# lunarlab-gatech/SLIDE_SLAM

Hardware: AMD Instinct MI355X
Metric: pose-graph updates/sec + ms/Gauss-Newton iter, 8-robot 10k-landmark graph (higher is better)
Workload: dtype f64

## Files before the change

slide_slam_amd/csrc/chol_kernels.hip:

```cpp
#include <hip/hip_runtime.h>
#include <stdlib.h>
#include <algorithm>
#include <type_traits>
#include <utility>
#include <vector>

#include "graph_dev.hpp"
#include "kernels.hpp"

namespace sl {

typedef double v4d __attribute__((ext_vector_type(4)));
constexpr int CHOL_BATCH_MAX = 8;
__device__ inline v4d mfma_f64(double a, double b, v4d c) { return __builtin_amdgcn_mfma_f64_16x16x4f64(a, b, c, 0, 0, 0); }

__device__ inline double rsqrt_nr(double d) {
#ifdef SLIDE_RSQRT_OLD
  double y = __builtin_amdgcn_rsq(d);
  y = y * (1.5 - 0.5 * d * y * y);
  y = y * (1.5 - 0.5 * d * y * y);
  return y;
#else
  double y = __builtin_amdgcn_rsq(d);
  double t = d * y, h = 0.5 * y;
// ... 1712 lines not shown
  }
}

extern "C" int slide_debug_pair_timeouts() {
  int v = -1;
  if (hipMemcpyFromSymbol(&v, HIP_SYMBOL(g_pair_timeouts), sizeof(int)) != hipSuccess) return -1;
  return v;
}
#ifdef SLIDE_STAMPS
extern "C" void slide_debug_stamps(unsigned long long* out) { (void)hipMemcpyFromSymbol(out, HIP_SYMBOL(g_stamps), sizeof(g_stamps)); }
extern "C" void slide_debug_chain_stamps(unsigned long long* out) { (void)hipMemcpyFromSymbol(out, HIP_SYMBOL(g_chain_stamps), sizeof(g_chain_stamps)); }
#endif

constexpr unsigned long long BWD_SENT = CHAIN_SENTINEL;

__global__ void k_chol_extract_y(const double* __restrict__ S, int ld, int T, int Tr, double* __restrict__ yv, double* __restrict__ dp, int* status,
                                 double* __restrict__ prev) {
  const int c = blockIdx.x * blockDim.x + threadIdx.x;
  if (c == 0) status[4] = 0;
  if (c < T * NB) {
    yv[c] = S[(size_t)c * ld + (size_t)Tr * NB];
    if (prev) prev[c] = dp[c];
    dp[c] = __longlong_as_double((long long)BWD_SENT);
  }
}

struct ExtractArgs { int n; const double* S[CHOL_STEP_BATCH_MAX]; int ld[CHOL_STEP_BATCH_MAX]; int T[CHOL_STEP_BATCH_MAX]; int Tr[CHOL_STEP_BATCH_MAX]; double* yv[CHOL_STEP_BATCH_MAX]; double* dp[CHOL_STEP_BATCH_MAX]; int* status[CHOL_STEP_BATCH_MAX]; };
__global__ void k_chol_extract_y_b(ExtractArgs A) {
  const int r = blockIdx.y;
  const int c = blockIdx.x * blockDim.x + threadIdx.x;
  if (c == 0) A.status[r][4] = 0;
  if (c < A.T[r] * NB) {
    A.yv[r][c] = A.S[r][(size_t)c * A.ld[r] + (size_t)A.Tr[r] * NB];
    A.dp[r][c] = __longlong_as_double((long long)BWD_SENT);
  }
}

constexpr int CHAIN_THREADS = 320;
struct alignas(16) ChainLds {
// ... 599 lines not shown
                            hipStream_t s) {
  const int nT = T * NB;
  for (int k = row0 / NB; k < T; ++k)
    hipLaunchKernelGGL(k_cov_fwd, dim3((unsigned)(T - k)), dim3(256), 0, s, S, ld, k, Ld + (size_t)k * NB * NB, Winv + (size_t)k * 1024, Y, nT);
  hipLaunchKernelGGL(k_cov_gram, dim3(1), dim3(256), 0, s, Y, nT, row0 / NB * NB, cov36);
}

struct SyrkArgs {
  int n;
  const double* S[CHOL_BATCH_MAX]; int ld[CHOL_BATCH_MAX]; int T[CHOL_BATCH_MAX]; int nbr[CHOL_BATCH_MAX];
  int b0[CHOL_BATCH_MAX];
  double* bord[CHOL_BATCH_MAX]; int ldb[CHOL_BATCH_MAX]; const int* bfirst[CHOL_BATCH_MAX];
  const double* bsrc[CHOL_BATCH_MAX];
  int ks; double* scratch;
  size_t scratch_stride;
  int ks_sys[2];
  const int* jobs;
  const int* segtab[CHOL_BATCH_MAX];
};
template <int RD>
__device__ __forceinline__ void border_syrk_body(const SyrkArgs& A) {
  int r = A.ks > 1 ? 0 : blockIdx.z, ib = blockIdx.x, jb = blockIdx.y;
  const int q = A.ks > 1 ? blockIdx.z : 0;
  if (A.jobs) {
    const int j = A.jobs[blockIdx.x];
    r = j >> 20; ib = (j >> 10) & 1023; jb = j & 1023;
  }
  const int nbr = A.nbr[r];
  if (ib > nbr || jb >= nbr || ib < jb) return;
  const int T = A.T[r], ld = A.ld[r];
  int ldb = A.ldb[r];
  int c0 = 0, c1 = T;
  const int* st = A.segtab[r];
  const int nseg = st ? st[0] : 1;
  if (!st && A.bfirst[r]) c0 = max(A.bfirst[r][ib], A.bfirst[r][jb]);
  int ksr = A.ks;
  if (A.ks > 1) {
    if (A.scratch_stride && r < 2 && A.ks_sys[r] > 0) ksr = A.ks_sys[r];
    if (q >= ksr) return;
    const int len = (T - c0 + ksr - 1) / ksr;
    c0 += q * len;
    c1 = min(T, c0 + len);
  }
  const double* bsrc = A.bsrc[r];
  if (!st && c0 >= c1 && !(bsrc && q == 0)) return;
  const double* S = A.S[r];
  const int wq = threadIdx.x >> 6, lane = threadIdx.x & 63, lr = lane & 15, lk = lane >> 4;
  const int ch = (wq >> 1) & 1, rh = wq & 1;
  if (A.jobs && ib == nbr && rh == 1 && !bsrc) return;
  const int B0 = A.b0[r];
  const double* pj0 = S + (size_t)lk * ld + (size_t)(B0 + jb) * NB + 32 * ch + 2 * lr;
  const double* pi0 = S + (size_t)lk * ld + (size_t)(B0 + ib) * NB + 32 * rh + 2 * lr;
  double* cbh = A.bord[r] + (size_t)(jb * NB + 32 * ch + 2 * lk) * ldb + (size_t)ib * NB + 32 * rh + 2 * lr;
  const double* cin = bsrc ? bsrc + (size_t)(jb * NB + 32 * ch + 2 * lk) * ldb + (size_t)ib * NB + 32 * rh + 2 * lr : cbh;
  const int ldin = ldb;
  if (q > 0) {
    ldb = NB;
    cbh = A.scratch + (size_t)r * A.scratch_stride + ((size_t)(jb * (nbr + 1) + ib) * (ksr - 1) + (q - 1)) * (NB * NB) + (size_t)(32 * ch + 2 * lk) * NB + 32 * rh + 2 * lr;
  }
  int total = 0;
  if (st) {
    for (int sg = 0; sg < nseg; ++sg) {
      const int* sf = st + 1 + nseg + sg * (nbr + 1);
      const int a0 = max(sf[ib], sf[jb]), a1 = st[1 + sg];
      if (a0 < a1) total += (a1 - a0) * 16;
    }
  } else {
    total = c1 > c0 ? (c1 - c0) * 16 : 0;
  }
  int sg_next = 0, rem = 0, issued = 0;
  const double *lpj = pj0, *lpi = pi0;
  v2d pa[RD], pb[RD];
  auto issue = [&](v2d& ra, v2d& rb) {
// ... 51 lines not shown
    for (int e = 0; e < 4; ++e) {
      v2d c2;
      c2[0] = acc[a][0][e]; c2[1] = acc[a][1][e];
      *(v2d*)(cbh + (size_t)(8 * e + a) * ldb) = c2;
    }
}
__global__ __launch_bounds__(256) void k_border_syrk(SyrkArgs A) { border_syrk_body<16>(A); }
__global__ __launch_bounds__(256) void k_border_syrk_rd8(SyrkArgs A) { border_syrk_body<8>(A); }
__global__ __launch_bounds__(256) void k_border_syrk_rd4(SyrkArgs A) { border_syrk_body<4>(A); }
static void launch_syrk_kernel(dim3 grid, size_t lds, hipStream_t s, const SyrkArgs& A) {
  static const int rd = getenv("SLIDE_SYRK_RD") ? atoi(getenv("SLIDE_SYRK_RD")) : 16;
  if (rd == 4) hipLaunchKernelGGL(k_border_syrk_rd4, grid, dim3(256), lds, s, A);
  else if (rd == 8) hipLaunchKernelGGL(k_border_syrk_rd8, grid, dim3(256), lds, s, A);
  else hipLaunchKernelGGL(k_border_syrk, grid, dim3(256), lds, s, A);
}
__global__ __launch_bounds__(256) void k_border_syrk_reduce(double* __restrict__ bord, int ldb, int nbr, int ks, const double* __restrict__ scratch,
                                                            const int* __restrict__ bfirst, int T) {
  const int ib = blockIdx.x >> 4, jb = blockIdx.y;
  if (ib > nbr || jb >= nbr || ib < jb) return;
  int c0 = 0;
  if (bfirst) c0 = max(bfirst[ib], bfirst[jb]);
  const int len = (T - c0 + ks - 1) / ks;
  const int e = (blockIdx.x & 15) * 256 + threadIdx.x;
  const int col = e / NB, row = e - col * NB;
  double* dst = bord + (size_t)(jb * NB + col) * ldb + (size_t)ib * NB + row;
  double v = *dst;
  for (int q = 1; q < ks; ++q)
    if (c0 + q * len < T) v += scratch[((size_t)(jb * (nbr + 1) + ib) * (ks - 1) + (q - 1)) * (NB * NB) + (size_t)col * NB + row];
  *dst = v;
}
__global__ __launch_bounds__(256) void k_border_syrk_reduce2(double* __restrict__ bordA, int ldbA, const double* __restrict__ bordB, int ldbB, int nbr,
                                                             int ksA, int ksB, const double* __restrict__ scratchA, const double* __restrict__ scratchB,
                                                             int TA, int TB) {
  const int ib = blockIdx.x >> 4, jb = blockIdx.y;
  if (ib > nbr || jb >= nbr || ib < jb) return;
  const int e = (blockIdx.x & 15) * 256 + threadIdx.x;
  const int col = e / NB, row = e - col * NB;
  double* dst = bordA + (size_t)(jb * NB + col) * ldbA + (size_t)ib * NB + row;
  double va = *dst, vb = bordB[(size_t)(jb * NB + col) * ldbB + (size_t)ib * NB + row];
  const int lenA = (TA + ksA - 1) / ksA, lenB = (TB + ksB - 1) / ksB;
  for (int q = 1; q < ksA; ++q)
    if (q * lenA < TA) va += scratchA[((size_t)(jb * (nbr + 1) + ib) * (ksA - 1) + (q - 1)) * (NB * NB) + (size_t)col * NB + row];
  for (int q = 1; q < ksB; ++q)
    if (q * lenB < TB) vb += scratchB[((size_t)(jb * (nbr + 1) + ib) * (ksB - 1) + (q - 1)) * (NB * NB) + (size_t)col * NB + row];
  *dst = va + vb;
}
void launch_border_syrk(const CholSystem* d, int n, hipStream_t s, double* scratch, int ks) {
  SyrkArgs A{};
  A.n = n;
  int nb = 0;
  for (int i = 0; i < n; ++i) {
    A.S[i] = d[i].S; A.ld[i] = d[i].ld; A.T[i] = d[i].T; A.nbr[i] = d[i].nbr; A.bord[i] = d[i].bord; A.ldb[i] = d[i].ldb; A.bfirst[i] = d[i].bfirst; A.bsrc[i] = d[i].bord_src;
    A.segtab[i] = d[i].segtab; A.b0[i] = d[i].b0 > 0 ? d[i].b0 : d[i].T;
    nb = d[i].nbr > nb ? d[i].nbr : nb;
  }
  if (nb <= 0) return;
  if (scratch && n == 1 && ks > 1) {
    A.ks = ks; A.scratch = scratch;
    launch_syrk_kernel(dim3(nb + 1, nb, ks), 0, s, A);
    hipLaunchKernelGGL(k_border_syrk_reduce, dim3(16 * (nb + 1), nb), dim3(256), 0, s, d[0].bord, d[0].ldb, d[0].nbr, ks, scratch, d[0].bfirst, d[0].T);
    return;
  }
  A.ks = 1; A.scratch = nullptr;
  launch_syrk_kernel(dim3(nb + 1, nb, n), 0, s, A);
}
void launch_border_syrk_jobs(const CholSystem* d, int n, const int* jobs, int njobs, int lds_pad, hipStream_t s, double* scratch, int ks, int jb_end,
                             const int* ks_sys, bool fuse_add) {
  SyrkArgs A{};
  A.n = n;
  for (int i = 0; i < n; ++i) {
    A.S[i] = d[i].S; A.ld[i] = d[i].ld; A.T[i] = d[i].T; A.nbr[i] = d[i].nbr; A.bord[i] = d[i].bord; A.ldb[i] = d[i].ldb; A.bfirst[i] = d[i].bfirst; A.bsrc[i] = d[i].bord_src;
    A.segtab[i] = d[i].segtab; A.b0[i] = d[i].b0 > 0 ? d[i].b0 : d[i].T;
  }
  if (njobs <= 0) return;
  A.ks = 1; A.scratch = nullptr; A.jobs = jobs;
// ... 3 lines not shown
    A.ks = km; A.scratch = scratch; A.scratch_stride = std::max<size_t>(1, (size_t)(nb + 1) * nb * (km - 1) * NB * NB);
    A.ks_sys[0] = ka; A.ks_sys[1] = kb;
    launch_syrk_kernel(dim3(njobs, 1, km), lds_pad, s, A);
    hipLaunchKernelGGL(k_border_syrk_reduce2, dim3(16 * (nb + 1), jb_end >= 0 ? jb_end : nb), dim3(256), 0, s, d[0].bord, d[0].ldb, d[1].bord, d[1].ldb, nb,
                       ka, kb, scratch, scratch + A.scratch_stride, d[0].T, d[1].T);
    return;
  }
  if (scratch && n == 1 && ks > 1) {
    A.ks = ks; A.scratch = scratch;
    launch_syrk_kernel(dim3(njobs, 1, ks), lds_pad, s, A);
    const int nb = d[0].nbr;
    hipLaunchKernelGGL(k_border_syrk_reduce, dim3(16 * (nb + 1), jb_end >= 0 ? jb_end : nb), dim3(256), 0, s, d[0].bord, d[0].ldb, nb, ks, scratch, d[0].bfirst, d[0].T);
    return;
  }
  launch_syrk_kernel(dim3(njobs), lds_pad, s, A);
}
struct BorderApplyArgs {
  int n;
  const double* S[CHOL_BATCH_MAX]; int ld[CHOL_BATCH_MAX]; int T[CHOL_BATCH_MAX]; int nbr[CHOL_BATCH_MAX]; int b0[CHOL_BATCH_MAX];
  double* yv[CHOL_BATCH_MAX]; const double* x[CHOL_BATCH_MAX];
  const int* segtab[CHOL_BATCH_MAX];
};
__global__ __launch_bounds__(256) void k_border_apply(BorderApplyArgs A) {
  const int r = blockIdx.z;
  const int col = blockIdx.x * 4 + (threadIdx.x >> 6), lane = threadIdx.x & 63;
  if (col >= A.T[r] * NB) return;
  const int nrow = A.nbr[r] * NB;
  const double* w = A.S[r] + (size_t)col * A.ld[r] + (size_t)A.b0[r] * NB;
  const double* x = A.x[r];
  double acc = 0.0;
// ... 491 lines not shown
```

slide_slam_amd/csrc/host_graph.hip:

```cpp
#include <chrono>

#include "host_graph.hpp"

#include <algorithm>
#include <cmath>
#include <cstdio>
#include <cstdlib>
#include <map>
#include <unordered_map>

namespace sl {

static inline int lam_ks_cap(int nl) {
  const int tiles = (nl + 1) * nl;
  if (tiles <= 0) return 1;
  return tiles <= 32 ? 16 : std::max(1, std::min(16, 256 / tiles));
}

thread_local std::string g_last_error;
void thread_capture_mode_local() {
  thread_local bool done = false;
  if (done) return;
  hipStreamCaptureMode m = hipStreamCaptureModeThreadLocal;
  (void)hipThreadExchangeStreamCaptureMode(&m);
// ... 777 lines not shown
  c.Ld = sep_Ld + (size_t)TL * NB * NB; c.Winv = sep_Winv + (size_t)TL * 1024; c.yv = sep_yv + (size_t)TL * NB; c.dp = sep_dp + (size_t)TL * NB;
  c.status = sep_status; c.nbr = sep_nl;
  if (!sep_dissected() && sep_prof_on) c.h_prof = h_sep_prof.data();
  return c;
}
void CholBatch::free_separator() {
  free_ll_sep_plans();
  if (sepS) (void)hipFree(sepS);
  sepS = nullptr; sep_len = 0;
  for (double** p : {&sep_Ld, &sep_Winv, &sep_yv, &sep_dp, &sep_bord, &lamS, &lam_Ld, &lam_Winv, &lam_yv, &lam_dp, &lam_scratch}) if (*p) { (void)hipFree(*p); *p = nullptr; }
  for (int** p : {&sep_status, &sep_ctr, &d_sep_off, &lam_status, &lam_ctr, &d_sep_prof, &d_leaf_prof, &sep_ctr2, &d_sep_jobs, &d_sep_tmask}) if (*p) { (void)hipFree(*p); *p = nullptr; }
  if (sep_scratch) { (void)hipFree(sep_scratch); sep_scratch = nullptr; }
  for (double** p : {&sep_top2, &sep_bord2}) if (*p) { (void)hipFree(*p); *p = nullptr; }
  if (d_sep_jobs2) { (void)hipFree(d_sep_jobs2); d_sep_jobs2 = nullptr; }
  if (d_lam_jobs2) { (void)hipFree(d_lam_jobs2); d_lam_jobs2 = nullptr; }
  sep_cap = 0; lam_cap = -1;
}
void CholBatch::set_segments(int n) {
  std::lock_guard<std::mutex> pl(pass_mtx);
  exact_serial = 0;
  std::vector<HostGraph*> gs;
  {
    std::lock_guard<std::mutex> lk(mtx);
    n_seg = n < 1 ? 1 : (n > 8 ? 8 : n);
    pass_dirty = true;
    gs.assign(graphs.begin(), graphs.end());
  }
  for (HostGraph* g : gs)
    if (g) { std::lock_guard<std::mutex> gl(g->mtx); g->topo_dirty = true; }
}
// ... 154 lines not shown
    for (int jb = 0; jb < Tt; ++jb)
      for (int ib = jb; ib <= nb; ++ib) codes.push_back(ib << 10 | jb);
    n_sep_jobs = (int)codes.size();
    SL_HIP(hipMalloc(reinterpret_cast<void**>(&d_sep_jobs), codes.size() * sizeof(int)));
    SL_HIP(hipMemcpyAsync(d_sep_jobs, codes.data(), codes.size() * sizeof(int), hipMemcpyHostToDevice, master)); SL_HIP(hipStreamSynchronize(master));
    sep_ks = std::max(1, std::min({8, TL / 4, (1024 + n_sep_jobs - 1) / std::max(n_sep_jobs, 1)}));
    if (getenv("SLIDE_SEP_KS")) sep_ks = std::max(1, std::min(16, atoi(getenv("SLIDE_SEP_KS"))));
    {
      std::vector<int> codes2;
      for (int sy = 0; sy < 2; ++sy)
        for (int c : codes) codes2.push_back(sy << 20 | c);
      if (d_sep_jobs2) { SL_HIP(hipFree(d_sep_jobs2)); d_sep_jobs2 = nullptr; }
      n_sep_jobs2 = (int)codes2.size();
      SL_HIP(hipMalloc(reinterpret_cast<void**>(&d_sep_jobs2), codes2.size() * sizeof(int)));
      SL_HIP(hipMemcpyAsync(d_sep_jobs2, codes2.data(), codes2.size() * sizeof(int), hipMemcpyHostToDevice, master)); SL_HIP(hipStreamSynchronize(master));
    }
    if (sep_ks > 1) {
      const size_t len = 2 * (size_t)(nb + 1) * nb * (sep_ks - 1) * NB * NB * sizeof(double);
      SL_HIP(hipMalloc(reinterpret_cast<void**>(&sep_scratch), len));
      SL_HIP(hipMemsetAsync(sep_scratch, 0, len, master)); SL_HIP(hipStreamSynchronize(master));
    }
    for (double** p : {&sep_top2, &sep_bord2}) if (*p) { SL_HIP(hipFree(*p)); *p = nullptr; }
    sep_ld2 = (Tt + sep_nl + 1) * NB;
    SL_HIP(hipMalloc(reinterpret_cast<void**>(&sep_top2), (size_t)sep_ld2 * Tt * NB * sizeof(double)));
    SL_HIP(hipMemsetAsync(sep_top2, 0, (size_t)sep_ld2 * Tt * NB * sizeof(double), master));
    if (sep_nl > 0) {
      const size_t nb2 = (size_t)(sep_nl + 1) * NB * sep_nl * NB;
      SL_HIP(hipMalloc(reinterpret_cast<void**>(&sep_bord2), nb2 * sizeof(double)));
      SL_HIP(hipMemsetAsync(sep_bord2, 0, nb2 * sizeof(double), master));
    }
// ... 147 lines not shown
          CholSystem tp2[2] = {top, top};
          for (int hh = 0; hh < 2; ++hh) {
            tp2[hh].S = sepS + (size_t)(hh ? sTa : 0) * NB * ld_s; tp2[hh].T = sep_leafT[hh]; tp2[hh].b0 = sTL;
            if (hh) { tp2[hh].bord = sep_top2; tp2[hh].ldb = sep_ld2; }
          }
          CholSystem sl2[2];
          int ks_lam[2] = {1, 1};
          for (int hh = 0; hh < 2 && sep_nl > 0; ++hh) {
            CholSystem sl{};
            sl.S = sepS + (size_t)(hh ? sTa : 0) * NB * ld_s; sl.ld = ld_s; sl.T = sep_leafT[hh]; sl.b0 = sep_Ts; sl.nbr = sep_nl;
            sl.bord = hh ? sep_bord2 : sep_bord; sl.ldb = (sep_nl + 1) * NB;
            ks_lam[hh] = std::max(1, std::min(lam_ks_cap(sep_nl), sep_leafT[hh] / 2));
            sl2[hh] = sl;
          }
          if (sep_scratch && (sep_nl == 0 || (lam_scratch && d_lam_jobs2))) {
            launch_border_syrk_jobs(tp2, 2, d_sep_jobs2, n_sep_jobs2, 0, master, sep_scratch, sep_ks, Tt, nullptr, true);
            if (sep_nl > 0) launch_border_syrk_jobs(sl2, 2, d_lam_jobs2, n_lam_jobs2, 0, master, lam_scratch, 1, -1, ks_lam, true);
          } else {
            for (int hh = 0; hh < 2; ++hh) {
              launch_border_syrk_jobs(&tp2[hh], 1, d_sep_jobs, n_sep_jobs, 0, master, sep_scratch, sep_ks, Tt);
              if (sep_nl > 0) launch_border_syrk(&sl2[hh], 1, master, lam_scratch, ks_lam[hh]);
            }
            launch_sep_top_add(Y, sTL, sep_top2, sep_ld2, sep_bord2, master);
          }
        } else {
          launch_border_syrk_jobs(&top, 1, d_sep_jobs, n_sep_jobs, 0, master, sep_scratch, sep_ks, Tt);
        }
      }
      if (ll_top) {
        const CholSystem ts = sep_top_system();
        launch_chol_ll(ll_top, &ts, 1, master);
      } else if ((chol_pair_mask() & 8) && d_pair_tickets) {
// ... 12 lines not shown
      const CholSystem ts = sep_top_system();
      launch_chol_batch(&ts, 1, sep_ctr, master, nullptr, false, 100, pair_tickets(11));
    } else {
      for (int k = 0; k < sep_Ts; ++k)
        launch_chol_step(sepS, ld_s, k, sep_Ts, sep_Ld + (size_t)k * NB * NB, sep_Winv + (size_t)k * 1024, sep_status, sep_ctr, nullptr,
                         sep_prof_on ? h_sep_prof.data() : nullptr, master, sep_nl);
      launch_chol_extract_y(sepS, ld_s, sep_Ts, sep_yv, sep_dp, sep_status, master, sep_nl);
    }
    if (sep_nl > 0) {
      CholSystem ss{};
      ss.S = sepS; ss.ld = ld_s; ss.T = sep_Ts; ss.yv = sep_yv; ss.nbr = sep_nl; ss.bord = sep_bord; ss.ldb = (sep_nl + 1) * NB; ss.bfirst = nullptr;
      CholSystem sr = ss;
      static const bool env_canon3 = !(getenv("SLIDE_SEP_CANONICAL") && getenv("SLIDE_SEP_CANONICAL")[0] == '0');
      if (owned || (whole && sep_dissected() && env_canon3 && n <= 8)) { sr.S = sepS + (size_t)sTL * NB * ld_s; sr.T = sTt; sr.b0 = sep_Ts; }
      const int ks = std::max(1, std::min(lam_ks_cap(sep_nl), sr.T / 2));
      launch_border_syrk(&sr, 1, master, lam_scratch, ks);
      launch_lam_prepare(sep_bord, sep_nl, sep_lam, lamS, master);
      const int ld_l = (sep_nl + 1) * NB;
      for (int k = 0; k < sep_nl; ++k)
        launch_chol_step(lamS, ld_l, k, sep_nl, lam_Ld + (size_t)k * NB * NB, lam_Winv + (size_t)k * 1024, lam_status, lam_ctr, nullptr, nullptr, master);
      launch_chol_extract_y(lamS, ld_l, sep_nl, lam_yv, lam_dp, lam_status, master);
      launch_chol_bwd_all(lamS, ld_l, sep_nl, lam_Ld, lam_Winv, lam_yv, lam_dp, lam_status, nullptr, master);
      const double* xl = lam_dp;
      if (!owned) launch_border_apply(&ss, 1, &xl, master);
      else {
        CholSystem ap2[2] = {ss, ss};
        ap2[0].S = sepS + (size_t)own_t0 * NB * ld_s; ap2[0].T = own_T; ap2[0].b0 = sep_Ts; ap2[0].yv = sep_yv + (size_t)own_t0 * NB;
        ap2[1].S = sepS + (size_t)sTL * NB * ld_s; ap2[1].T = sTt; ap2[1].b0 = sep_Ts; ap2[1].yv = sep_yv + (size_t)sTL * NB;
        const double* xl2[2] = {xl, xl};
        launch_border_apply(ap2, 2, xl2, master);
      }
    }
    if (sep_dissected()) {
      double* St = sepS + (size_t)sTL * NB * ld_s + (size_t)sTL * NB;
      launch_chol_bwd_all(St, ld_s, sTt, sep_Ld + (size_t)sTL * NB * NB, sep_Winv + (size_t)sTL * 1024, sep_yv + (size_t)sTL * NB, sep_dp + (size_t)sTL * NB,
                          sep_status, nullptr, master);
      launch_ints_clear(sep_status + 4, 1, master);
// ... 1689 lines not shown
```

slide_slam_amd/csrc/host_graph.hpp:

```cpp
#pragma once
#include <hip/hip_runtime.h>

#include <cstdint>
#include <cstring>
#include <condition_variable>
#include <functional>
#include <mutex>
#include <string>
#include <unordered_map>
#include <vector>

#include "../../include/slide_gpu.h"
#include "graph_dev.hpp"
#include "host_layout.hpp"
#include "kernels.hpp"
#include "sl_math.hpp"

namespace sl {

extern thread_local std::string g_last_error;
void thread_capture_mode_local();
bool hip_ok(hipError_t e, const char* what);
inline bool robot_ok(int r) { return r >= 0 && r < SLIDE_MAX_ROBOTS; }
int decode_status(const int* st8);
// ... 222 lines not shown
  double* sep_x = nullptr; long long sep_x_len = 0;
  int sep_m = 0, sep_Ts = 0;
  double *sep_Ld = nullptr, *sep_Winv = nullptr, *sep_yv = nullptr, *sep_dp = nullptr;
  int *sep_status = nullptr, *sep_ctr = nullptr, *d_sep_off = nullptr;
  int sep_cap = 0;
  std::vector<int> h_sep_prof; int* d_sep_prof = nullptr; bool sep_prof_on = false;
  int sep_leafT[2] = {0, 0}, sep_used[2] = {0, 0};
  int sep_owner = -1; bool sep_leader = true;
  std::vector<int> h_leaf_prof[2];
  int* d_leaf_prof = nullptr;
  int* d_sep_tmask = nullptr;
  int* sep_ctr2 = nullptr; int* d_sep_jobs = nullptr; int n_sep_jobs = 0; double* sep_scratch = nullptr; int sep_ks = 1;
  double *sep_top2 = nullptr, *sep_bord2 = nullptr; int sep_ld2 = 0; unsigned sep_mask_b = 0;
  int* d_lam_jobs2 = nullptr; int n_lam_jobs2 = 0;
  int* d_sep_jobs2 = nullptr; int n_sep_jobs2 = 0;
  bool sep_dissected() const { return sep_leafT[0] > 0 && sep_leafT[1] > 0; }
  int sep_lam = 0, sep_nl = 0, lam_cap = -1;
  double *lam_scratch = nullptr;
  double *sep_bord = nullptr, *lamS = nullptr, *lam_Ld = nullptr, *lam_Winv = nullptr, *lam_yv = nullptr, *lam_dp = nullptr;
  int *lam_status = nullptr, *lam_ctr = nullptr;
  SepLayout sep_layout() const {
    SepLayout Y{sepS, sep_bord, sep_x, sep_Ts, sep_nl, sep_m, sep_lam, {0, 0, 0, 0}, 0, 0};
    if (sep_dissected()) {
      Y.gap[0] = sep_used[0]; Y.gap[1] = sep_leafT[0] * NB;
      Y.gap[2] = sep_leafT[0] * NB + sep_used[1]; Y.gap[3] = (sep_leafT[0] + sep_leafT[1]) * NB;
      Y.hTa = sep_leafT[0]; Y.hTL = sep_leafT[0] + sep_leafT[1];
    }
    return Y;
  }
  int prepare_separator();
// ... 391 lines not shown
```

slide_slam_amd/csrc/kernels.hpp:

```cpp
#pragma once
#include <hip/hip_runtime.h>
#include <stdint.h>
#include <vector>

#include "graph_dev.hpp"
#include "sl_math.hpp"

namespace sl {

void init_solver_kernels();
void launch_relin(const GraphDev& G, hipStream_t s);
void launch_linearize(const GraphDev& G, const ObsLossDev& O, hipStream_t s);
void launch_observation_weights(const GraphDev& G, const ObsLossDev& O, bool robust, int n, double* out2n, hipStream_t s);
void launch_observation_weights_batched(const GraphDev* d, const ObsLossDev* dO, bool robust, const int* off, const int* cnt, int n, double* out2n,
                                        hipStream_t s);
void launch_robust_reweight(const GraphDev& G, const RobustDev& R, hipStream_t s);
void launch_closure_weights(const GraphDev& G, const RobustDev& R, const int* idx, int n, double* out2n, hipStream_t s);
void launch_robust_reweight_batched(const GraphDev* d, const RobustDev* dR, const GraphDev* h, int n, hipStream_t s);
void launch_closure_weights_batched(const GraphDev* d, const RobustDev* dR, const int* ent2, int n, double* out2n, hipStream_t s);
void launch_landmark(const GraphDev& G, int mode, hipStream_t s);
void launch_pose(const GraphDev& G, hipStream_t s);
void launch_schur(const GraphDev& G, hipStream_t s);
void launch_backsub(const GraphDev& G, int mode, hipStream_t s);
void launch_shared_pack(const GraphDev& G, int what, double* buf, hipStream_t s);
// ... 15 lines not shown
void launch_phase2_batched(const GraphDev* d, const GraphDev* h, int n, double* const* bufs, hipStream_t s);
void launch_phase3_batched(const GraphDev* d, const GraphDev* h, int n, double* const* bufs, hipStream_t s);
void launch_ghost_exchange(const GraphDev& G, int what, double* buf, hipStream_t s);
void launch_ghost_exchange_batched(const GraphDev* d, int n, int n_gslots, int what, double* const* bufs, hipStream_t s);
void launch_border_assemble_batched(const GraphDev* d, const GraphDev* h, int n, hipStream_t s, bool clear = true, bool fills = true);
void launch_sep_extract_batched(const GraphDev* d, const GraphDev* h, int n, const int* n_sep_poses, hipStream_t s);
void launch_sep_pose_scatter_batched(const GraphDev* d, const GraphDev* h, int n, double* const* xloc, hipStream_t s);
struct SepLayout { double* sys; double* bord; double* packed; int Ts, nl, ms, lam; int gap[4]; int hTa, hTL; };
void launch_ghost_refresh_local(const GraphDev* d, int n, int n_gslots, hipStream_t s);
void launch_copy_pairs(const double* const* src, double* const* dst, const int* count, int n, hipStream_t s);
void launch_sep_gather(const GraphDev* h, int n, const int* const* maps, const SepLayout& Y, bool packed, hipStream_t s, const int* tmask = nullptr,
                       int split_col = -1, unsigned mask_b = 0, double* sys2 = nullptr, int ld2 = 0, double* bord2 = nullptr);
void launch_sep_top_add(const SepLayout& Y, int c0, const double* sys2, int ld2, const double* bord2, hipStream_t s);
void launch_sep_unpack(const SepLayout& Y, hipStream_t s, int c0 = 0, int c1 = -1, bool to_packed = false);
void launch_lam_prepare(const double* bord, int nl, int lam, double* out, hipStream_t s);
void launch_sep_xloc(int n, const int* const* maps, int ms, int lam, const double* xs, const double* xl, double* const* xloc, hipStream_t s);
void launch_arrow_finish_batched(const GraphDev* d, const GraphDev* h, int n, const double* xs, const int* sep_off, hipStream_t s, bool slots_onto);
struct AsmMerge { int mask; };
AsmMerge asm_merge_env();
void launch_phase3_arrow_batched(const GraphDev* d, const GraphDev* h, int n, hipStream_t s);

void launch_chol_step(double* S, int ld, int k, int T, double* Ld, double* Winv, int* status, int* ctr, float* L32, const int* h_prof, hipStream_t s, int nbr = 0);
void launch_chol_extract_y(const double* S, int ld, int T, double* yv, double* dp, int* status, hipStream_t s, int nbr = 0, int b0 = 0, double* prev = nullptr);
constexpr unsigned long long CHAIN_SENTINEL = 0x7FF8DEADBEEF0BADull;
struct CholSystem { double* S; int ld, T; double* Ld; double* Winv; double* yv; double* dp; int* status;
                    float* L32;
                    const int* h_prof;
                    const int* prof; const int* first;
                    double* ctab;
                    int nbr;
// ... 13 lines not shown
  ~CholPlanHook();
  CholPlanHook(const CholPlanHook&) = delete;
  CholPlanHook& operator=(const CholPlanHook&) = delete;
private:
  CholPlanHook* prev;
};
int chol_device_cus();
bool chol_pair_supported(const CholSystem* d, int n);
void launch_chol_bwd_batch(const CholSystem* d, int n, hipStream_t s);
struct CholLLPlan;
CholLLPlan* chol_ll_plan_create(const CholSystem* d, int n, const int* const* h_ord = nullptr, hipStream_t upload_stream = nullptr);
void chol_ll_plan_destroy(CholLLPlan* p);
int chol_ll_plan_tasks(const CholLLPlan* p);
int chol_ll_plan_columns(const CholLLPlan* p);
void launch_chol_ll(const CholLLPlan* p, const CholSystem* d, int n, hipStream_t s, int* trace = nullptr);
void launch_border_syrk(const CholSystem* d, int n, hipStream_t s, double* scratch = nullptr, int ks = 1);
void launch_border_syrk_jobs(const CholSystem* d, int n, const int* jobs, int njobs, int lds_pad, hipStream_t s, double* scratch = nullptr, int ks = 1, int jb_end = -1,
                             const int* ks_sys = nullptr, bool fuse_add = false);
void launch_border_apply(const CholSystem* d, int n, const double* const* xloc, hipStream_t s);
void launch_chain_batch(const CholSystem* d, int n, const double* const* in, double* const* out, bool fwd, bool f32, bool prepared,
                        double* const* next_out, hipStream_t s);
void launch_chain_tables(const CholSystem* d, int n, hipStream_t s);
void launch_chol_bwd_all(const double* S, int ld, int T, const double* Ld, const double* Winv, double* yv, double* dp, int* status, const int* prof, hipStream_t s,
                         const double* wf_prev = nullptr, double wf_thr = 0.0, int wf_Tprev = 0, int wf_lim = -1);
void launch_pose_covariance(const double* S, int ld, int T, const double* Ld, const double* Winv, double* Y, int row0, double* cov36,
                            hipStream_t s);
void launch_selected_inverse(const double* S, int ld, int T, const double* Ld, const double* Winv, const int* prof, const int* d_prof,
                             double* Sg, double* Z, hipStream_t s);
void launch_selected_inverse_prep(const double* S, int ld, int T, const double* Ld, const double* Winv, const int* prof, const int* d_prof,
                                  double* Sg, double* Z, hipStream_t s);
void launch_pose_blocks(const double* Sg, int ld, const int* poses, int n, double* out, hipStream_t s, const int* prow = nullptr);
void launch_landmark_covariances(const GraphDev& G, const double* Sg, int ld, const int* lids, int n, double* out, hipStream_t s,
                                 const int* prow = nullptr);
// ... 248 lines not shown
```

slide_slam_amd/csrc/solver_kernels.hip:

```cpp
#include <hip/hip_runtime.h>
#include <algorithm>
#include <cstring>

#include "graph_dev.hpp"
#include "kernels.hpp"
#include "sl_math.hpp"

namespace sl {

struct BufPtrs { double* p[8]; };

__device__ inline void pose_retract12(const double* in12, const double* d6, int chart, double* out12) {
  to12(retract(from12(in12), d6, chart), out12);
}
__device__ inline void lm_retract(int type, const double* in, const double* d, int chart, double* out) {
  if (type == VT_POINT) {
    out[0] = in[0] + d[0]; out[1] = in[1] + d[1]; out[2] = in[2] + d[2];
  } else if (type == VT_CUBE) {
    pose_retract12(in, d, chart, out);
    out[12] = in[12] + d[6]; out[13] = in[13] + d[7]; out[14] = in[14] + d[8];
  } else {
    out[3] = in[3] + d[0]; out[4] = in[4] + d[1]; out[5] = in[5] + d[2];
    out[0] = in[0] + d[3]; out[1] = in[1] + d[4]; out[2] = in[2] + d[5];
    out[6] = in[6] + d[6];
// ... 1563 lines not shown
      else A.bord2[(size_t)(vc - NL) * ((size_t)(Y.nl + 1) * NB) + (vr - NL)] = s2;
    }
  }
}
__global__ __launch_bounds__(256) void k_sep_unpack(SepLayout Y, int c0, int c1, int to_packed) {
  const int vr = blockIdx.x * 256 + threadIdx.x, vc = c0 * NB + blockIdx.y;
  const int NT = (Y.Ts + Y.nl) * NB;
  if (vr > NT || vc >= NT || vc >= c1 * NB || vr < vc / NB * NB) return;
  if (sep_packed_hole(vr, vc, Y.hTa, Y.hTL)) return;
  if (to_packed) { *sep_slot(Y, vr, vc, true) = *sep_slot(Y, vr, vc, false); return; }
  double v = *sep_slot(Y, vr, vc, true);
  if (vr == vc && ((vc >= Y.gap[0] && vc < Y.gap[1]) || (vc >= Y.gap[2] && vc < Y.gap[3]))) v = 1.0;
  *sep_slot(Y, vr, vc, false) = v;
}
__global__ __launch_bounds__(256) void k_lam_prepare(const double* __restrict__ bord, int nl, int lam, double* __restrict__ out) {
  const int r = blockIdx.x * 256 + threadIdx.x, c = blockIdx.y;
  const int NT = nl * NB, ld = (nl + 1) * NB;
  if (r > NT || c >= NT) return;
  const bool rhs = r == NT;
  if (!rhs && r < c) return;
  double v;
  if (c < lam && (rhs || r < lam)) v = -bord[(size_t)c * ld + r];
  else v = (r == c) ? 1.0 : 0.0;
  out[(size_t)c * ld + r] = v;
}
struct SepScatterArgs { int n, m, ms; const double* xs; const double* xl; double* xloc[8]; const int* map[8]; };
__global__ __launch_bounds__(256) void k_sep_xloc(SepScatterArgs A) {
  const int g = blockIdx.x * 256 + threadIdx.x, r = blockIdx.y;
  if (g >= A.m || r >= A.n) return;
  const int lc = A.map[r][g];
  if (lc >= 0) A.xloc[r][lc] = g < A.ms ? A.xs[g] : A.xl[g - A.ms];
}
__global__ __launch_bounds__(256) void k_sep_lm_delta_b(const GraphDev* __restrict__ Gs, SepScatterArgs A, const int* __restrict__ sep_off) {
  const GraphDev G = Gs[blockIdx.z];
  const int t = blockIdx.x * 256 + threadIdx.x;
  const int sidx = t / 9, k = t - 9 * sidx;
  if (sidx >= G.n_slots) return;
  const int l = G.sh_lid[sidx];
  if (l < 0) return;
// ... 585 lines not shown
```

Before: 4115.

## Fuse lambda-system syrk with top pairs and single-block lambda solve

Merges the border SYRK for the two top systems and the two lambda systems into one launch over a combined job list, with a paired reduce kernel handling both. For a one-block lambda system, the reduce, prepare, Cholesky step, y-extract and backward solve are folded into a single 512-thread kernel in place of a chain of small launches. The goal is to cut kernel-launch and serialization overhead on tiny systems. The cost is a single-block kernel with low parallelism and extra scratch indexing, both gated by an env mask that is on by default.

```diff
diff --git a/slide_slam_amd/csrc/chol_kernels.hip b/slide_slam_amd/csrc/chol_kernels.hip
--- a/slide_slam_amd/csrc/chol_kernels.hip
+++ b/slide_slam_amd/csrc/chol_kernels.hip
@@ -1750,15 +1750,18 @@
 
 constexpr unsigned long long BWD_SENT = CHAIN_SENTINEL;
 
-__global__ void k_chol_extract_y(const double* __restrict__ S, int ld, int T, int Tr, double* __restrict__ yv, double* __restrict__ dp, int* status,
-                                 double* __restrict__ prev) {
-  const int c = blockIdx.x * blockDim.x + threadIdx.x;
+__device__ __forceinline__ void extract_y_elem(const double* __restrict__ S, int ld, int T, int Tr, double* __restrict__ yv, double* __restrict__ dp,
+                                               int* status, double* __restrict__ prev, int c) {
   if (c == 0) status[4] = 0;
   if (c < T * NB) {
     yv[c] = S[(size_t)c * ld + (size_t)Tr * NB];
     if (prev) prev[c] = dp[c];
     dp[c] = __longlong_as_double((long long)BWD_SENT);
   }
+}
+__global__ void k_chol_extract_y(const double* __restrict__ S, int ld, int T, int Tr, double* __restrict__ yv, double* __restrict__ dp, int* status,
+                                 double* __restrict__ prev) {
+  extract_y_elem(S, ld, T, Tr, yv, dp, status, prev, blockIdx.x * blockDim.x + threadIdx.x);
 }
 
 struct ExtractArgs { int n; const double* S[CHOL_STEP_BATCH_MAX]; int ld[CHOL_STEP_BATCH_MAX]; int T[CHOL_STEP_BATCH_MAX]; int Tr[CHOL_STEP_BATCH_MAX]; double* yv[CHOL_STEP_BATCH_MAX]; double* dp[CHOL_STEP_BATCH_MAX]; int* status[CHOL_STEP_BATCH_MAX]; };
@@ -2388,7 +2391,8 @@
   const double* bsrc[CHOL_BATCH_MAX];
   int ks; double* scratch;
   size_t scratch_stride;
-  int ks_sys[2];
+  int ks_sys[4];
+  double* scratch2; size_t scratch_stride2;
   const int* jobs;
   const int* segtab[CHOL_BATCH_MAX];
 };
@@ -2410,7 +2414,7 @@
   if (!st && A.bfirst[r]) c0 = max(A.bfirst[r][ib], A.bfirst[r][jb]);
   int ksr = A.ks;
   if (A.ks > 1) {
-    if (A.scratch_stride && r < 2 && A.ks_sys[r] > 0) ksr = A.ks_sys[r];
+    if (A.scratch_stride && r < 4 && A.ks_sys[r] > 0) ksr = A.ks_sys[r];
     if (q >= ksr) return;
     const int len = (T - c0 + ksr - 1) / ksr;
     c0 += q * len;
@@ -2430,7 +2434,8 @@
   const int ldin = ldb;
   if (q > 0) {
     ldb = NB;
-    cbh = A.scratch + (size_t)r * A.scratch_stride + ((size_t)(jb * (nbr + 1) + ib) * (ksr - 1) + (q - 1)) * (NB * NB) + (size_t)(32 * ch + 2 * lk) * NB + 32 * rh + 2 * lr;
+    double* sc = r < 2 ? A.scratch + (size_t)r * A.scratch_stride : A.scratch2 + (size_t)(r - 2) * A.scratch_stride2;
+    cbh = sc + ((size_t)(jb * (nbr + 1) + ib) * (ksr - 1) + (q - 1)) * (NB * NB) + (size_t)(32 * ch + 2 * lk) * NB + 32 * rh + 2 * lr;
   }
   int total = 0;
   if (st) {
@@ -2512,27 +2517,51 @@
   else if (rd == 8) hipLaunchKernelGGL(k_border_syrk_rd8, grid, dim3(256), lds, s, A);
   else hipLaunchKernelGGL(k_border_syrk, grid, dim3(256), lds, s, A);
 }
-__global__ __launch_bounds__(256) void k_border_syrk_reduce(double* __restrict__ bord, int ldb, int nbr, int ks, const double* __restrict__ scratch,
-                                                            const int* __restrict__ bfirst, int T) {
-  const int ib = blockIdx.x >> 4, jb = blockIdx.y;
+template <int N>
+__device__ __forceinline__ void border_reduce_elems(double* __restrict__ bord, int ldb, int nbr, int ks, const double* __restrict__ scratch,
+                                                    const int* __restrict__ bfirst, int T, int ib, int jb, int e0, int stride) {
   if (ib > nbr || jb >= nbr || ib < jb) return;
   int c0 = 0;
   if (bfirst) c0 = max(bfirst[ib], bfirst[jb]);
   const int len = (T - c0 + ks - 1) / ks;
-  const int e = (blockIdx.x & 15) * 256 + threadIdx.x;
-  const int col = e / NB, row = e - col * NB;
-  double* dst = bord + (size_t)(jb * NB + col) * ldb + (size_t)ib * NB + row;
-  double v = *dst;
-  for (int q = 1; q < ks; ++q)
-    if (c0 + q * len < T) v += scratch[((size_t)(jb * (nbr + 1) + ib) * (ks - 1) + (q - 1)) * (NB * NB) + (size_t)col * NB + row];
-  *dst = v;
-}
-__global__ __launch_bounds__(256) void k_border_syrk_reduce2(double* __restrict__ bordA, int ldbA, const double* __restrict__ bordB, int ldbB, int nbr,
-                                                             int ksA, int ksB, const double* __restrict__ scratchA, const double* __restrict__ scratchB,
-                                                             int TA, int TB) {
-  const int ib = blockIdx.x >> 4, jb = blockIdx.y;
+  double* dst[N];
+  double v[N];
+#pragma unroll
+  for (int u = 0; u < N; ++u) {
+    const int e = e0 + u * stride;
+    const int col = e / NB, row = e - col * NB;
+    dst[u] = bord + (size_t)(jb * NB + col) * ldb + (size_t)ib * NB + row;
+    v[u] = *dst[u];
+  }
+  int nq = ks;
+  while (nq > 1 && c0 + (nq - 1) * len >= T) --nq;
+  const double* sq = scratch + (size_t)(jb * (nbr + 1) + ib) * (ks - 1) * (NB * NB) + e0;
+  int q = 1;
+  for (; q + 1 < nq; q += 2) {
+    double p[N], p2[N];
+#pragma unroll
+    for (int u = 0; u < N; ++u) { p[u] = sq[(size_t)(q - 1) * (NB * NB) + u * stride]; p2[u] = sq[(size_t)q * (NB * NB) + u * stride]; }
+#pragma unroll
+    for (int u = 0; u < N; ++u) { v[u] += p[u]; v[u] += p2[u]; }
+  }
+  if (q < nq) {
+    double p[N];
+#pragma unroll
+    for (int u = 0; u < N; ++u) p[u] = sq[(size_t)(q - 1) * (NB * NB) + u * stride];
+#pragma unroll
+    for (int u = 0; u < N; ++u) v[u] += p[u];
+  }
+#pragma unroll
+  for (int u = 0; u < N; ++u) *dst[u] = v[u];
+}
+__global__ __launch_bounds__(256) void k_border_syrk_reduce(double* __restrict__ bord, int ldb, int nbr, int ks, const double* __restrict__ scratch,
+                                                            const int* __restrict__ bfirst, int T) {
+  border_reduce_elems<1>(bord, ldb, nbr, ks, scratch, bfirst, T, blockIdx.x >> 4, blockIdx.y, (blockIdx.x & 15) * 256 + threadIdx.x, 0);
+}
+__device__ __forceinline__ void border_reduce2_elem(double* __restrict__ bordA, int ldbA, const double* __restrict__ bordB, int ldbB, int nbr,
+                                                    int ksA, int ksB, const double* __restrict__ scratchA, const double* __restrict__ scratchB,
+                                                    int TA, int TB, int ib, int jb, int e) {
   if (ib > nbr || jb >= nbr || ib < jb) return;
-  const int e = (blockIdx.x & 15) * 256 + threadIdx.x;
   const int col = e / NB, row = e - col * NB;
   double* dst = bordA + (size_t)(jb * NB + col) * ldbA + (size_t)ib * NB + row;
   double va = *dst, vb = bordB[(size_t)(jb * NB + col) * ldbB + (size_t)ib * NB + row];
@@ -2543,7 +2572,48 @@
     if (q * lenB < TB) vb += scratchB[((size_t)(jb * (nbr + 1) + ib) * (ksB - 1) + (q - 1)) * (NB * NB) + (size_t)col * NB + row];
   *dst = va + vb;
 }
-void launch_border_syrk(const CholSystem* d, int n, hipStream_t s, double* scratch, int ks) {
+__global__ __launch_bounds__(256) void k_border_syrk_reduce2(double* __restrict__ bordA, int ldbA, const double* __restrict__ bordB, int ldbB, int nbr,
+                                                             int ksA, int ksB, const double* __restrict__ scratchA, const double* __restrict__ scratchB,
+                                                             int TA, int TB) {
+  border_reduce2_elem(bordA, ldbA, bordB, ldbB, nbr, ksA, ksB, scratchA, scratchB, TA, TB, blockIdx.x >> 4, blockIdx.y,
+                      (blockIdx.x & 15) * 256 + threadIdx.x);
+}
+struct Reduce2Pair { double* bordA; const double* bordB; const double* scratchA; const double* scratchB; int ldbA, ldbB, nbr, jb_end, ksA, ksB, TA, TB; };
+struct Reduce2Args { Reduce2Pair p[2]; };
+__global__ __launch_bounds__(256) void k_border_syrk_reduce2p(Reduce2Args A) {
+  const Reduce2Pair& P = A.p[blockIdx.z];
+  if ((int)blockIdx.y >= P.jb_end) return;
+  border_reduce2_elem(P.bordA, P.ldbA, P.bordB, P.ldbB, P.nbr, P.ksA, P.ksB, P.scratchA, P.scratchB, P.TA, P.TB, blockIdx.x >> 4, blockIdx.y,
+                      (blockIdx.x & 15) * 256 + threadIdx.x);
+}
+union LamSolveLds { ALds a; ChainLds c; };
+__global__ __launch_bounds__(512) void k_lam_solve1(double* bord, int ks, const double* __restrict__ scratch, int Tsum, int lam, double* S,
+                                                    double* Ld, double* Winv, double* yv, double* dp, int* status, int* ctr) {
+  __shared__ LamSolveLds U;
+  constexpr int ld = 2 * NB;
+  const int tid = threadIdx.x;
+  if (ks > 1) border_reduce_elems<16>(bord, ld, 1, ks, scratch, nullptr, Tsum, tid >> 8, 0, tid & 255, 256);
+  __syncthreads();
+  if (tid < 7 * (NB + 1)) lam_prepare_elems<10>(bord, 1, lam, S, tid % (NB + 1), tid / (NB + 1), 7);
+  if (tid == 0) ctr[1] = 0;
+  __syncthreads();
+  step_type_a(S, ld, 0, 1, 1, 0, -1, Ld, Winv, status, U.a, nullptr, 0, 0);
+  __syncthreads();
+  extract_y_elem(S, ld, 1, 1, yv, dp, status, nullptr, tid);
+  __syncthreads();
+  if (tid == 0) status[4] = 1;
+  bwd_chain_body<false>(U.c, S, ld, 1, Ld, Winv, yv, dp, status, 0, nullptr, nullptr);
+}
+void launch_lam_solve1(double* bord, int ks, const double* scratch, int Tsum, int lam, double* S, double* Ld, double* Winv, double* yv, double* dp,
+                       int* status, int* ctr, hipStream_t s) {
+  hipLaunchKernelGGL(k_lam_solve1, dim3(1), dim3(512), 0, s, bord, scratch ? ks : 1, scratch, Tsum, lam, S, Ld, Winv, yv, dp, status, ctr);
+}
+LamFuse lam_fuse_env() {
+  LamFuse F{3};
+  if (const char* e = getenv("SLIDE_LAM_FUSE")) F.mask = atoi(e);
+  return F;
+}
+void launch_border_syrk(const CholSystem* d, int n, hipStream_t s, double* scratch, int ks, bool reduce) {
   SyrkArgs A{};
   A.n = n;
   int nb = 0;
@@ -2556,7 +2626,7 @@
   if (scratch && n == 1 && ks > 1) {
     A.ks = ks; A.scratch = scratch;
     launch_syrk_kernel(dim3(nb + 1, nb, ks), 0, s, A);
-    hipLaunchKernelGGL(k_border_syrk_reduce, dim3(16 * (nb + 1), nb), dim3(256), 0, s, d[0].bord, d[0].ldb, d[0].nbr, ks, scratch, d[0].bfirst, d[0].T);
+    if (reduce) hipLaunchKernelGGL(k_border_syrk_reduce, dim3(16 * (nb + 1), nb), dim3(256), 0, s, d[0].bord, d[0].ldb, d[0].nbr, ks, scratch, d[0].bfirst, d[0].T);
     return;
   }
   A.ks = 1; A.scratch = nullptr;
@@ -2590,6 +2660,29 @@
     return;
   }
   launch_syrk_kernel(dim3(njobs), lds_pad, s, A);
+}
+void launch_border_syrk_pairs(const CholSystem* top, const CholSystem* lam, const int* jobs, int njobs, hipStream_t s, double* scratch_top,
+                              int ks_top, int jb_end, double* scratch_lam, const int* ks_lam) {
+  if (njobs <= 0) return;
+  SyrkArgs A{};
+  A.n = 4;
+  for (int i = 0; i < 4; ++i) {
+    const CholSystem& d = i < 2 ? top[i] : lam[i - 2];
+    A.S[i] = d.S; A.ld[i] = d.ld; A.T[i] = d.T; A.nbr[i] = d.nbr; A.bord[i] = d.bord; A.ldb[i] = d.ldb; A.bfirst[i] = d.bfirst; A.bsrc[i] = d.bord_src;
+    A.segtab[i] = d.segtab; A.b0[i] = d.b0 > 0 ? d.b0 : d.T;
+  }
+  A.jobs = jobs;
+  const int nbt = top[0].nbr, nbl = lam[0].nbr;
+  const int kt = std::max(1, ks_top), ka = std::max(1, ks_lam[0]), kb = std::max(1, ks_lam[1]), kl = std::max(ka, kb), km = std::max(kt, kl);
+  A.ks = km;
+  A.scratch = scratch_top; A.scratch_stride = std::max<size_t>(1, (size_t)(nbt + 1) * nbt * (kt - 1) * NB * NB);
+  A.scratch2 = scratch_lam; A.scratch_stride2 = std::max<size_t>(1, (size_t)(nbl + 1) * nbl * (kl - 1) * NB * NB);
+  A.ks_sys[0] = A.ks_sys[1] = kt; A.ks_sys[2] = ka; A.ks_sys[3] = kb;
+  launch_syrk_kernel(dim3(njobs, 1, km), 0, s, A);
+  Reduce2Args R{};
+  R.p[0] = {top[0].bord, top[1].bord, scratch_top, scratch_top + A.scratch_stride, top[0].ldb, top[1].ldb, nbt, jb_end, kt, kt, top[0].T, top[1].T};
+  R.p[1] = {lam[0].bord, lam[1].bord, scratch_lam, scratch_lam + A.scratch_stride2, lam[0].ldb, lam[1].ldb, nbl, nbl, ka, kb, lam[0].T, lam[1].T};
+  hipLaunchKernelGGL(k_border_syrk_reduce2p, dim3(16 * (std::max(nbt, nbl) + 1), std::max(jb_end, nbl), 2), dim3(256), 0, s, R);
 }
 struct BorderApplyArgs {
   int n;
diff --git a/slide_slam_amd/csrc/host_graph.hip b/slide_slam_amd/csrc/host_graph.hip
--- a/slide_slam_amd/csrc/host_graph.hip
+++ b/slide_slam_amd/csrc/host_graph.hip
@@ -815,6 +815,7 @@
   for (double** p : {&sep_top2, &sep_bord2}) if (*p) { (void)hipFree(*p); *p = nullptr; }
   if (d_sep_jobs2) { (void)hipFree(d_sep_jobs2); d_sep_jobs2 = nullptr; }
   if (d_lam_jobs2) { (void)hipFree(d_lam_jobs2); d_lam_jobs2 = nullptr; }
+  if (d_sep_jobs4) { (void)hipFree(d_sep_jobs4); d_sep_jobs4 = nullptr; }
   sep_cap = 0; lam_cap = -1;
 }
 void CholBatch::set_segments(int n) {
@@ -999,6 +1000,16 @@
       n_sep_jobs2 = (int)codes2.size();
       SL_HIP(hipMalloc(reinterpret_cast<void**>(&d_sep_jobs2), codes2.size() * sizeof(int)));
       SL_HIP(hipMemcpyAsync(d_sep_jobs2, codes2.data(), codes2.size() * sizeof(int), hipMemcpyHostToDevice, master)); SL_HIP(hipStreamSynchronize(master));
+      if (d_sep_jobs4) { SL_HIP(hipFree(d_sep_jobs4)); d_sep_jobs4 = nullptr; }
+      n_sep_jobs4 = 0;
+      if (sep_nl > 0) {
+        for (int sy = 2; sy < 4; ++sy)
+          for (int jb = 0; jb < sep_nl; ++jb)
+            for (int ib = jb; ib <= sep_nl; ++ib) codes2.push_back(sy << 20 | ib << 10 | jb);
+        n_sep_jobs4 = (int)codes2.size();
+        SL_HIP(hipMalloc(reinterpret_cast<void**>(&d_sep_jobs4), codes2.size() * sizeof(int)));
+        SL_HIP(hipMemcpyAsync(d_sep_jobs4, codes2.data(), codes2.size() * sizeof(int), hipMemcpyHostToDevice, master)); SL_HIP(hipStreamSynchronize(master));
+      }
     }
     if (sep_ks > 1) {
       const size_t len = 2 * (size_t)(nb + 1) * nb * (sep_ks - 1) * NB * NB * sizeof(double);
@@ -1176,8 +1187,12 @@
             sl2[hh] = sl;
           }
           if (sep_scratch && (sep_nl == 0 || (lam_scratch && d_lam_jobs2))) {
-            launch_border_syrk_jobs(tp2, 2, d_sep_jobs2, n_sep_jobs2, 0, master, sep_scratch, sep_ks, Tt, nullptr, true);
-            if (sep_nl > 0) launch_border_syrk_jobs(sl2, 2, d_lam_jobs2, n_lam_jobs2, 0, master, lam_scratch, 1, -1, ks_lam, true);
+            if (sep_nl > 0 && d_sep_jobs4 && (lam_fuse_env().mask & 1)) {
+              launch_border_syrk_pairs(tp2, sl2, d_sep_jobs4, n_sep_jobs4, master, sep_scratch, sep_ks, Tt, lam_scratch, ks_lam);
+            } else {
+              launch_border_syrk_jobs(tp2, 2, d_sep_jobs2, n_sep_jobs2, 0, master, sep_scratch, sep_ks, Tt, nullptr, true);
+              if (sep_nl > 0) launch_border_syrk_jobs(sl2, 2, d_lam_jobs2, n_lam_jobs2, 0, master, lam_scratch, 1, -1, ks_lam, true);
+            }
           } else {
             for (int hh = 0; hh < 2; ++hh) {
               launch_border_syrk_jobs(&tp2[hh], 1, d_sep_jobs, n_sep_jobs, 0, master, sep_scratch, sep_ks, Tt);
@@ -1220,13 +1235,18 @@
       static const bool env_canon3 = !(getenv("SLIDE_SEP_CANONICAL") && getenv("SLIDE_SEP_CANONICAL")[0] == '0');
       if (owned || (whole && sep_dissected() && env_canon3 && n <= 8)) { sr.S = sepS + (size_t)sTL * NB * ld_s; sr.T = sTt; sr.b0 = sep_Ts; }
       const int ks = std::max(1, std::min(lam_ks_cap(sep_nl), sr.T / 2));
-      launch_border_syrk(&sr, 1, master, lam_scratch, ks);
-      launch_lam_prepare(sep_bord, sep_nl, sep_lam, lamS, master);
-      const int ld_l = (sep_nl + 1) * NB;
-      for (int k = 0; k < sep_nl; ++k)
-        launch_chol_step(lamS, ld_l, k, sep_nl, lam_Ld + (size_t)k * NB * NB, lam_Winv + (size_t)k * 1024, lam_status, lam_ctr, nullptr, nullptr, master);
-      launch_chol_extract_y(lamS, ld_l, sep_nl, lam_yv, lam_dp, lam_status, master);
-      launch_chol_bwd_all(lamS, ld_l, sep_nl, lam_Ld, lam_Winv, lam_yv, lam_dp, lam_status, nullptr, master);
+      if (sep_nl == 1 && (lam_fuse_env().mask & 2)) {
+        launch_border_syrk(&sr, 1, master, lam_scratch, ks, false);
+        launch_lam_solve1(sep_bord, ks, lam_scratch, sr.T, sep_lam, lamS, lam_Ld, lam_Winv, lam_yv, lam_dp, lam_status, lam_ctr, master);
+      } else {
+        launch_border_syrk(&sr, 1, master, lam_scratch, ks);
+        launch_lam_prepare(sep_bord, sep_nl, sep_lam, lamS, master);
+        const int ld_l = (sep_nl + 1) * NB;
+        for (int k = 0; k < sep_nl; ++k)
+          launch_chol_step(lamS, ld_l, k, sep_nl, lam_Ld + (size_t)k * NB * NB, lam_Winv + (size_t)k * 1024, lam_status, lam_ctr, nullptr, nullptr, master);
+        launch_chol_extract_y(lamS, ld_l, sep_nl, lam_yv, lam_dp, lam_status, master);
+        launch_chol_bwd_all(lamS, ld_l, sep_nl, lam_Ld, lam_Winv, lam_yv, lam_dp, lam_status, nullptr, master);
+      }
       const double* xl = lam_dp;
       if (!owned) launch_border_apply(&ss, 1, &xl, master);
       else {
diff --git a/slide_slam_amd/csrc/host_graph.hpp b/slide_slam_amd/csrc/host_graph.hpp
--- a/slide_slam_amd/csrc/host_graph.hpp
+++ b/slide_slam_amd/csrc/host_graph.hpp
@@ -260,6 +260,7 @@
   double *sep_top2 = nullptr, *sep_bord2 = nullptr; int sep_ld2 = 0; unsigned sep_mask_b = 0;
   int* d_lam_jobs2 = nullptr; int n_lam_jobs2 = 0;
   int* d_sep_jobs2 = nullptr; int n_sep_jobs2 = 0;
+  int* d_sep_jobs4 = nullptr; int n_sep_jobs4 = 0;
   bool sep_dissected() const { return sep_leafT[0] > 0 && sep_leafT[1] > 0; }
   int sep_lam = 0, sep_nl = 0, lam_cap = -1;
   double *lam_scratch = nullptr;
diff --git a/slide_slam_amd/csrc/kernels.hpp b/slide_slam_amd/csrc/kernels.hpp
--- a/slide_slam_amd/csrc/kernels.hpp
+++ b/slide_slam_amd/csrc/kernels.hpp
@@ -53,6 +53,25 @@
 void launch_sep_top_add(const SepLayout& Y, int c0, const double* sys2, int ld2, const double* bord2, hipStream_t s);
 void launch_sep_unpack(const SepLayout& Y, hipStream_t s, int c0 = 0, int c1 = -1, bool to_packed = false);
 void launch_lam_prepare(const double* bord, int nl, int lam, double* out, hipStream_t s);
+template <int N>
+__device__ __forceinline__ void lam_prepare_elems(const double* __restrict__ bord, int nl, int lam, double* __restrict__ out, int r, int c0, int cstride) {
+  const int NT = nl * NB, ld = (nl + 1) * NB;
+  if (r > NT) return;
+  const bool rhs = r == NT;
+  double v[N];
+#pragma unroll
+  for (int u = 0; u < N; ++u) {
+    const int c = c0 + u * cstride;
+    const bool live = c < NT && (rhs || r >= c);
+    v[u] = (r == c) ? 1.0 : 0.0;
+    if (live && c < lam && (rhs || r < lam)) v[u] = -bord[(size_t)c * ld + r];
+  }
+#pragma unroll
+  for (int u = 0; u < N; ++u) {
+    const int c = c0 + u * cstride;
+    if (c < NT && (rhs || r >= c)) out[(size_t)c * ld + r] = v[u];
+  }
+}
 void launch_sep_xloc(int n, const int* const* maps, int ms, int lam, const double* xs, const double* xl, double* const* xloc, hipStream_t s);
 void launch_arrow_finish_batched(const GraphDev* d, const GraphDev* h, int n, const double* xs, const int* sep_off, hipStream_t s, bool slots_onto);
 struct AsmMerge { int mask; };
@@ -96,9 +115,15 @@
 int chol_ll_plan_tasks(const CholLLPlan* p);
 int chol_ll_plan_columns(const CholLLPlan* p);
 void launch_chol_ll(const CholLLPlan* p, const CholSystem* d, int n, hipStream_t s, int* trace = nullptr);
-void launch_border_syrk(const CholSystem* d, int n, hipStream_t s, double* scratch = nullptr, int ks = 1);
+void launch_border_syrk(const CholSystem* d, int n, hipStream_t s, double* scratch = nullptr, int ks = 1, bool reduce = true);
+struct LamFuse { int mask; };
+LamFuse lam_fuse_env();
+void launch_lam_solve1(double* bord, int ks, const double* scratch, int Tsum, int lam, double* S, double* Ld, double* Winv, double* yv, double* dp,
+                       int* status, int* ctr, hipStream_t s);
 void launch_border_syrk_jobs(const CholSystem* d, int n, const int* jobs, int njobs, int lds_pad, hipStream_t s, double* scratch = nullptr, int ks = 1, int jb_end = -1,
                              const int* ks_sys = nullptr, bool fuse_add = false);
+void launch_border_syrk_pairs(const CholSystem* top, const CholSystem* lam, const int* jobs, int njobs, hipStream_t s, double* scratch_top,
+                              int ks_top, int jb_end, double* scratch_lam, const int* ks_lam);
 void launch_border_apply(const CholSystem* d, int n, const double* const* xloc, hipStream_t s);
 void launch_chain_batch(const CholSystem* d, int n, const double* const* in, double* const* out, bool fwd, bool f32, bool prepared,
                         double* const* next_out, hipStream_t s);
diff --git a/slide_slam_amd/csrc/solver_kernels.hip b/slide_slam_amd/csrc/solver_kernels.hip
--- a/slide_slam_amd/csrc/solver_kernels.hip
+++ b/slide_slam_amd/csrc/solver_kernels.hip
@@ -1601,15 +1601,7 @@
   *sep_slot(Y, vr, vc, false) = v;
 }
 __global__ __launch_bounds__(256) void k_lam_prepare(const double* __restrict__ bord, int nl, int lam, double* __restrict__ out) {
-  const int r = blockIdx.x * 256 + threadIdx.x, c = blockIdx.y;
-  const int NT = nl * NB, ld = (nl + 1) * NB;
-  if (r > NT || c >= NT) return;
-  const bool rhs = r == NT;
-  if (!rhs && r < c) return;
-  double v;
-  if (c < lam && (rhs || r < lam)) v = -bord[(size_t)c * ld + r];
-  else v = (r == c) ? 1.0 : 0.0;
-  out[(size_t)c * ld + r] = v;
+  lam_prepare_elems<1>(bord, nl, lam, out, blockIdx.x * 256 + threadIdx.x, blockIdx.y, 0);
 }
 struct SepScatterArgs { int n, m, ms; const double* xs; const double* xl; double* xloc[8]; const int* map[8]; };
 __global__ __launch_bounds__(256) void k_sep_xloc(SepScatterArgs A) {
```

After: 4165, median of 6. 1.2% higher.
